# lzhangbj/ASVA

Measured on AMD Instinct MI355X. Metric: UNet denoising steps/sec, 12x256x256 bf16, CFG on, higher is better.
Workload: dtype bf16; 1 GPU; BASELINE configs[1]: AVSync15 shape, 1 clip(s) per GPU per forward, 12x256x256 (latent 12x32x32), SD1.5-shaped AudioUNet3D 1.17B params random-init, CFG batch 2 (audio guidance 4.0), DDIM-50 schedule, step = UNet forward + guidance + scheduler update; clips_per_gpu=1, unet_batch=2, frames=12, launch=hipGraph replay, parallelism=dp1 (independent clips)

## Files before the change

asva_amd/_lib.py:

```python
from __future__ import annotations

import ctypes as C
import os

import torch

from . import precision as P

_HERE = os.path.dirname(os.path.abspath(__file__))
LIB_PATH = os.environ.get("AVSD_LIB_PATH") or os.path.join(_HERE, "libavsd_hip.so")
LIB_PATHS = {"bf16": LIB_PATH, "fp16": os.environ.get("AVSD_LIB_PATH_F16") or os.path.join(_HERE, "libavsd_hip_f16.so")}

c_void_p, c_int, c_float, c_int64 = C.c_void_p, C.c_int, C.c_float, C.c_int64


class GemmDesc(C.Structure):

    _fields_ = [
        ("A", c_void_p), ("A2", c_void_p), ("W", c_void_p), ("out", c_void_p),
        ("bias", c_void_p), ("rowvec", c_void_p), ("res1", c_void_p), ("res2", c_void_p),
        ("M", C.c_int32), ("N", C.c_int32), ("K", C.c_int32),
        ("lda", C.c_int32), ("lda2", C.c_int32), ("k_split", C.c_int32), ("ldw", C.c_int32),
        ("ldc", C.c_int32), ("ldr1", C.c_int32), ("ldr2", C.c_int32),
        ("rows_per_vec", C.c_int32), ("ldv", C.c_int32),
# ... 14 lines not shown


class XAttnDesc(C.Structure):

    _fields_ = [
        ("h", c_void_p), ("ldh", C.c_int32), ("res_f32", C.c_int32),
        ("res", c_void_p), ("ldres", C.c_int32),
        ("M", C.c_int32), ("C", C.c_int32), ("heads", C.c_int32), ("L", C.c_int32),
        ("ln_stats", c_void_p), ("ln_eps", C.c_float), ("scale", C.c_float),
        ("wq", c_void_p), ("ldwq", C.c_int32), ("lk", C.c_int32),
        ("q_colsum", c_void_p), ("q_bias", c_void_p),
        ("k", c_void_p), ("vt", c_void_p),
        ("lk_pad", C.c_int32), ("q_per_kv", C.c_int32),
        ("wo", c_void_p), ("ldwo", C.c_int32), ("ldo", C.c_int32),
        ("o_bias", c_void_p), ("out", c_void_p),
        ("out_master", c_void_p), ("ldm", C.c_int32), ("reserved0", C.c_int32),
        ("rowstats", c_void_p),
        ("stats_pos", c_void_p), ("pos_hw", C.c_int32), ("pos_frames", C.c_int32),
    ]


SIGNATURES = {
    "avsd_abi_version": (c_int, []),
    "avsd_precision": (C.c_char_p, []),
    "avsd_last_error": (C.c_char_p, []),
    "avsd_device_info": (c_int, [C.c_char_p, c_int, C.POINTER(c_int)]),
    "avsd_gemm_bf16": (c_int, [C.POINTER(GemmDesc), c_void_p]),
    "avsd_sizeof_gemm_desc": (c_int, []),
    "avsd_cross_attention_block": (c_int, [C.POINTER(XAttnDesc), c_void_p]),
    "avsd_gemm_conv3r_supported": (c_int, [c_int, c_int, c_int, c_int]),
    "avsd_gemm_conv3r2d_supported": (c_int, [c_int, c_int, c_int, c_int]),
    "avsd_cross_attention_block_supported": (c_int, [c_int, c_int, c_int]),
    "avsd_sizeof_xattn_desc": (c_int, []),
    "avsd_linear_small_m": (c_int, [c_void_p, c_void_p, c_void_p, c_void_p, c_int, c_int, c_int, c_int, c_int, c_int, c_void_p]),
    "avsd_groupnorm_stats": (c_int, [c_void_p, c_int, c_int, c_void_p, c_int, c_int, c_int, c_int, c_int, c_void_p, c_int, c_void_p]),
    "avsd_groupnorm_apply": (c_int, [c_void_p, c_int, c_int, c_void_p, c_int, c_int, c_int, c_int, c_int, c_void_p, c_void_p, c_float,
                                     c_void_p, c_int, c_int, c_void_p, c_int, c_void_p]),
    "avsd_ln_fold": (c_int, [c_void_p, c_int, c_int, c_void_p, c_void_p]),
    "avsd_groupnorm_fused_supported": (c_int, [c_int, c_int, c_int, c_int, c_int, c_int]),
    "avsd_groupnorm_fused": (c_int, [c_void_p, c_int, c_int, c_void_p, c_int, c_int, c_int, c_int, c_int, c_void_p, c_void_p, c_float,
                                     c_int, c_void_p, c_int, c_void_p]),
    "avsd_groupnorm_nchunks": (c_int, [c_int, c_int, c_int]),
    "avsd_groupnorm_scratch_floats": (c_int, [c_int, c_int, c_int, c_int]),
    "avsd_layernorm": (c_int, [c_void_p, c_int, c_void_p, c_int, c_int, c_int, c_void_p, c_void_p, c_float, c_void_p, c_int, c_int, c_void_p]),
    "avsd_softmax_rows": (c_int, [c_void_p, c_int, c_void_p, c_int, c_int, c_int, c_void_p]),
    "avsd_attention": (c_int, [c_void_p, c_int, c_void_p, c_int, c_void_p, c_int, c_void_p, c_int, c_int, c_int, c_int, c_int,
                               c_int, c_int, c_int, c_void_p, c_int, c_float, c_void_p]),
    "avsd_attention_fp8": (c_int, [c_void_p, c_int, c_void_p, c_int, c_void_p, c_int, c_void_p, c_int, c_int, c_int, c_int, c_int,
                                   c_int, c_int, c_int, c_void_p, c_int, c_float, c_float, c_float, c_float, c_void_p]),
    "avsd_temporal_attention": (c_int, [c_void_p, c_int, c_void_p, c_int, c_int, c_int, c_int, c_int, c_int, c_float, c_void_p]),
    "avsd_ncfhw_to_rows": (c_int, [c_void_p, c_void_p, c_int, c_int, c_int, c_int, c_int, c_int, c_float, c_void_p]),
    "avsd_rows_to_ncfhw": (c_int, [c_void_p, c_int, c_void_p, c_int, c_int, c_int, c_int, c_void_p]),
    "avsd_timestep_embedding": (c_int, [c_void_p, c_void_p, c_int, c_int, c_void_p]),
    "avsd_guided_step": (c_int, [c_void_p, c_int, c_float, c_float, c_void_p, c_int, c_float, C.POINTER(C.c_int32), C.POINTER(C.c_float),
                                 c_int, c_void_p, c_void_p, c_float, c_float, c_int, c_int, c_int, c_int, c_void_p]),
    "avsd_guided_multistep": (c_int, [c_void_p, c_int, c_float, c_float, c_void_p, c_int, C.POINTER(C.c_int32), C.POINTER(C.c_float),
                                      c_int, c_void_p, c_void_p, c_float, c_float, c_float, c_float, c_int, c_int, c_int, c_int, c_void_p]),
    "avsd_vae_postprocess":(c_int, [c_void_p, c_int, c_void_p, c_int, c_int, c_void_p]),
    "avsd_vae_postprocess_u8": (c_int, [c_void_p, c_int, c_void_p, c_int, c_int, c_void_p]),
    "avsd_kaldi_fbank": (c_int, [c_void_p, c_int, c_int, C.c_int64, c_void_p, c_void_p, c_int, c_int, c_int, c_int, c_float, c_int,
                                 c_void_p, c_int, c_float, c_float, c_void_p]),
    "avsd_resample_sinc_f32": (c_int, [c_void_p, c_int, c_int, c_int64, c_void_p, c_int, c_int, c_int, c_void_p, c_int, c_int64, c_void_p]),
    "avsd_patchify": (c_int, [c_void_p, c_void_p, c_int, c_int, c_int, c_int, c_int, c_int, c_int, c_void_p]),
    "avsd_vit_tokens": (c_int, [c_void_p, c_void_p, c_void_p, c_void_p, c_int, c_int, c_int, c_int, c_void_p]),
    "avsd_copy": (c_int, [c_void_p, c_void_p, c_int64, c_int, c_void_p]),
    "avsd_xattn_pack_kv": (c_int, [c_void_p, c_int, c_int, c_int, c_void_p, c_int, c_int, c_void_p, c_void_p, c_int, c_void_p]),
# ... 99 lines not shown
```

asva_amd/build.py:

```python
from __future__ import annotations

import os
import subprocess
import sys
from concurrent.futures import ThreadPoolExecutor

HERE = os.path.dirname(os.path.abspath(__file__))
CSRC = os.path.join(HERE, "csrc")
OBJ = os.path.join(CSRC, "_obj")
LIB = os.path.join(HERE, "libavsd_hip.so")
VARIANTS = {"bf16": ("", LIB, []), "fp16": ("_f16", os.path.join(HERE, "libavsd_hip_f16.so"), ["-DAVSD_F16=1"])}
SOURCES = ["lib.hip", "attention.hip", "attention_x2.hip", "gemm_f32.hip", "gemm4.hip", "nstream.hip", "conv3r.hip", "norm.hip", "groupnorm_fused.hip", "elementwise.hip", "audio.hip", "xattn.hip", "attention_fp8.hip", "avsync.hip", "clip_text.hip", "imagebind_eval.hip", "plan.hip"]
GEMM_UNITS = 7
HEADERS = [os.path.join(CSRC, "avsd_common.h"), os.path.join(CSRC, "gemm_common.h"), os.path.join(CSRC, "gemm4_loops.inc"),
           os.path.join(HERE, "..", "include", "avsd.h")]
FLAGS = ["--offload-arch=gfx950", "-O3", "-std=c++17", "-fPIC", "-Wall", "-Wno-unused-function"]


PLAN_HOST = os.path.join(HERE, "plan_host")


def _hipcc() -> str:
    for cand in (os.environ.get("HIPCC"), "/opt/rocm/bin/hipcc", "hipcc"):
        if cand and (os.path.isabs(cand) and os.path.exists(cand) or not os.path.isabs(cand)):
            return cand
    raise RuntimeError("hipcc not found")


def _stale(target: str, deps: list[str]) -> bool:
    if not os.path.exists(target):
        return True
    t = os.path.getmtime(target)
    return any(os.path.getmtime(d) > t for d in deps)


def build(verbose: bool = False, force: bool = False, variants=("bf16", "fp16")) -> str:
    hipcc = _hipcc()
    jobs = []
    links = []
    for var in variants:
        suffix, lib, defs = VARIANTS[var]
        objdir = OBJ + suffix
        os.makedirs(objdir, exist_ok=True)
        objs = []
        stale = False
# ... 39 lines not shown
```

asva_amd/csrc/plan.hip:

```cpp
#include "avsd_common.h"

#include <stdio.h>
#include <string.h>

#include <string>
#include <type_traits>
#include <utility>
#include <vector>

namespace {

struct RArg {
  int64_t i = 0;
  double f = 0.0;
  void* p = nullptr;
};

template <class T>
T conv(const RArg& a) {
  if constexpr (std::is_pointer_v<T>) return reinterpret_cast<T>(a.p);
  else if constexpr (std::is_floating_point_v<T>) return static_cast<T>(a.f);
  else return static_cast<T>(a.i);
}
template <class... A, size_t... I>
int call_impl(int (*fn)(A...), const RArg* a, std::index_sequence<I...>) {
  return fn(conv<A>(a[I])...);
}
template <class... A>
int call(int (*fn)(A...), const RArg* a, int n, const char* name) {
  if (n != (int)sizeof...(A)) {
    avsd_set_error("plan: %s recorded with %d arguments, this library takes %d", name, n, (int)sizeof...(A));
    return AVSD_EINVAL;
  }
  return call_impl(fn, a, std::index_sequence_for<A...>{});
}

typedef int (*thunk_t)(const RArg*, int);
struct Entry {
  const char* name;
  thunk_t thunk;
  size_t desc_bytes;
};
#define AVSD_PLAN_ENTRY(fn) {#fn, [](const RArg* a, int n) { return call(&fn, a, n, #fn); }, 0}
#define AVSD_PLAN_ENTRY_DESC(fn, T) {#fn, [](const RArg* a, int n) { return call(&fn, a, n, #fn); }, sizeof(T)}
const Entry kEntries[] = {
    AVSD_PLAN_ENTRY_DESC(avsd_gemm_bf16, avsd_gemm_desc), AVSD_PLAN_ENTRY_DESC(avsd_cross_attention_block, avsd_xattn_desc), AVSD_PLAN_ENTRY(avsd_linear_small_m),
    AVSD_PLAN_ENTRY(avsd_groupnorm_stats),  AVSD_PLAN_ENTRY(avsd_groupnorm_apply),       AVSD_PLAN_ENTRY(avsd_layernorm),
    AVSD_PLAN_ENTRY(avsd_softmax_rows),     AVSD_PLAN_ENTRY(avsd_attention),             AVSD_PLAN_ENTRY(avsd_attention_fp8),
    AVSD_PLAN_ENTRY(avsd_temporal_attention), AVSD_PLAN_ENTRY(avsd_ncfhw_to_rows),       AVSD_PLAN_ENTRY(avsd_rows_to_ncfhw),
    AVSD_PLAN_ENTRY(avsd_timestep_embedding), AVSD_PLAN_ENTRY(avsd_guided_step),         AVSD_PLAN_ENTRY(avsd_vae_postprocess),
    AVSD_PLAN_ENTRY(avsd_vae_postprocess_u8), AVSD_PLAN_ENTRY(avsd_kaldi_fbank),         AVSD_PLAN_ENTRY(avsd_patchify),
    AVSD_PLAN_ENTRY(avsd_vit_tokens),       AVSD_PLAN_ENTRY(avsd_copy),                  AVSD_PLAN_ENTRY(avsd_xattn_pack_kv),
    AVSD_PLAN_ENTRY(avsd_linear_small_m_x2), AVSD_PLAN_ENTRY(avsd_groupnorm_stats_x2),   AVSD_PLAN_ENTRY(avsd_groupnorm_apply_x2),
    AVSD_PLAN_ENTRY(avsd_layernorm_x2),     AVSD_PLAN_ENTRY(avsd_attention_x2),          AVSD_PLAN_ENTRY(avsd_temporal_attention_x2),
    AVSD_PLAN_ENTRY(avsd_ncfhw_to_rows_x2), AVSD_PLAN_ENTRY(avsd_split_f32),             AVSD_PLAN_ENTRY(avsd_vae_postprocess_x2),
    AVSD_PLAN_ENTRY(avsd_vae_postprocess_u8_x2), AVSD_PLAN_ENTRY(avsd_softmax_rows_x2),
    AVSD_PLAN_ENTRY(avsd_groupnorm_fused),  AVSD_PLAN_ENTRY(avsd_groupnorm_fused_x2),
    AVSD_PLAN_ENTRY(avsd_ln_fold),          AVSD_PLAN_ENTRY(avsd_guided_multistep),
    AVSD_PLAN_ENTRY(avsd_convnd_f32),       AVSD_PLAN_ENTRY(avsd_maxpool_hw_f32),        AVSD_PLAN_ENTRY(avsd_mean_rows_f32),
    AVSD_PLAN_ENTRY(avsd_resize_aa_normalize_f32),
    AVSD_PLAN_ENTRY(avsd_convnd_ld_f32),    AVSD_PLAN_ENTRY(avsd_pool3_hw_f32),
    AVSD_PLAN_ENTRY(avsd_conv3d_same_f32),  AVSD_PLAN_ENTRY(avsd_maxpool3d_same_f32),
    AVSD_PLAN_ENTRY(avsd_embed_tokens_f32), AVSD_PLAN_ENTRY(avsd_layernorm_f32),         AVSD_PLAN_ENTRY(avsd_attention_causal_f32),
    AVSD_PLAN_ENTRY(avsd_quick_gelu_f32),
    AVSD_PLAN_ENTRY(avsd_attention_f32),    AVSD_PLAN_ENTRY(avsd_gelu_f32),              AVSD_PLAN_ENTRY(avsd_vit_tokens_f32),
    AVSD_PLAN_ENTRY(avsd_cosine_rows_f32),   AVSD_PLAN_ENTRY(avsd_normalize_rows_f32),
    AVSD_PLAN_ENTRY(avsd_resample_sinc_f32),
};

struct Reloc {
  uint32_t field_off;
  int32_t buf;
  int64_t off;
};
struct Arg {
  uint8_t tag = 0;
  int64_t i = 0;
  double f = 0.0;
  int32_t buf = -1;
  int64_t off = 0;
  std::vector<unsigned char> blob;
  std::vector<Reloc> relocs;
};
struct Call {
  thunk_t thunk = nullptr;
// ... 352 lines not shown
```

asva_amd/ops.py:

```python
from __future__ import annotations

import os
import ctypes as C
from typing import Optional

import torch

from . import _lib
from . import precision as P
from ._lib import GemmDesc, XAttnDesc, check

PLAIN, TMIX, CONV3 = 0, 1, 2
GEGLU, OUT_F32, GELU, XCD_N, ROWSTATS, LNFUSE, RES1_F32, RES2_F32, X2, KROT, W_FRAG, OUT_REST = 1, 2, 4, 8, 16, 32, 64, 128, 256, 512, 1024, 2048
_XCD_MODE = "auto"
F32 = torch.float32


class KernelTimer:

    def __init__(self):
        self.records = []
        self.replays = []

    def start(self):
# ... 954 lines not shown
    d.h, d.ldh = _p(h), _ld(h)
    _req(res, F32 if res.dtype == F32 else P.ACT, "res")
    d.res, d.ldres, d.res_f32 = _p(res), _ld(res), int(res.dtype == F32)
    d.M, d.C, d.heads, d.L = M, Cc, heads, L
    d.ln_stats, d.ln_eps = _p(stats), float(eps)
    d.scale = float(scale) if scale is not None else float(Cc // heads) ** -0.5
    d.wq, d.ldwq, d.q_colsum, d.q_bias = _p(wq), _ld(wq), _p(q_colsum), _p(q_bias)
    d.k, d.vt, d.lk, d.lk_pad, d.q_per_kv = _p(k), _p(vt), lk, lk_pad, q_per_kv
    d.wo, d.ldwo, d.o_bias = _p(wo), _ld(wo), _p(o_bias)
    d.out, d.ldo = _p(out), _ld(out)
    if master is not None:
        _req(master, F32, "master")
        d.out_master, d.ldm = _p(master), _ld(master)
    if rowstats is not None:
        _req(rowstats, F32, "rowstats")
        d.rowstats = _p(rowstats)
    if stats_pos is not None:
        tbl, hw_, fr_ = stats_pos
        _req(tbl, F32, "stats_pos")
        if rowstats is None or not tbl.is_contiguous() or tbl.shape != (fr_, Cc) or hw_ <= 0:
            raise ValueError("cross_attention_block: stats_pos = (f32 [frames, C], hw, frames) goes with rowstats")
        d.stats_pos, d.pos_hw, d.pos_frames = _p(tbl), int(hw_), int(fr_)
    ev = _TIMER.start() if _TIMER is not None else None
    check(_lib.lib().avsd_cross_attention_block(C.byref(d), _stream()), "avsd_cross_attention_block")
    if ev is not None:
        dc = XAttnDesc.from_buffer_copy(d)
        _TIMER.add_replay("cross_attention_block", lambda dc=dc: check(_lib.lib().avsd_cross_attention_block(C.byref(dc), _stream()),
                                                                         "avsd_cross_attention_block"),
                          (h, stats, wq, q_colsum, q_bias, k, vt, wo, o_bias, res, out, master, rowstats, stats_pos))
        _TIMER.stop(ev, "cross_attention_block", 4.0 * M * Cc * Cc + 4.0 * M * lk * Cc, _nbytes(h, out, res, master) + 4.0 * Cc * Cc)
    return out


def temporal_attention(qkv: torch.Tensor, *, b: int, frames: int, hw: int, heads: int,
                       scale: Optional[float] = None, out: Optional[torch.Tensor] = None) -> torch.Tensor:
    _req(qkv, P.ACT, "qkv")
    Cc = qkv.shape[1] // 3
    d = Cc // heads
    if out is None:
        out = alloc16((qkv.shape[0], Cc), qkv.device)
    if scale is None:
        scale = float(d) ** -0.5
    if P.SPLIT:
        a_ = (_p(qkv), _ld(qkv), _lo(qkv), _p(out), _ld(out), _lo(out), b, frames, hw, heads, d, float(scale))
        call = lambda: check(_lib.lib().avsd_temporal_attention_x2(*a_, _stream()), "avsd_temporal_attention_x2")
    else:
        a_ = (_p(qkv), _ld(qkv), _p(out), _ld(out), b, frames, hw, heads, d, float(scale))
        call = lambda: check(_lib.lib().avsd_temporal_attention(*a_, _stream()), "avsd_temporal_attention")
    _timed("temporal_attention", 4.0 * b * hw * heads * frames * frames * d, _nbytes(qkv, out), (qkv, out), call)
    return out


def ncfhw_to_rows(x: torch.Tensor, cpad: int, rep: int = 1, scale: float = 1.0) -> torch.Tensor:
    _req(x, F32, "x")
    if not x.is_contiguous():
        raise ValueError("ncfhw_to_rows: x must be contiguous")
    B, Cc, Fr, H, W = x.shape
    out = alloc16((rep * B * Fr * H * W, cpad), x.device)
    if P.SPLIT:
        check(_lib.lib().avsd_ncfhw_to_rows_x2(_p(x), _p(out), _lo(out), B, Cc, Fr, H * W, cpad, rep, float(scale), _stream()),
              "avsd_ncfhw_to_rows_x2")
        return out
    check(_lib.lib().avsd_ncfhw_to_rows(_p(x), _p(out), B, Cc, Fr, H * W, cpad, rep, float(scale), _stream()),
          "avsd_ncfhw_to_rows")
    return out

# ... 482 lines not shown
```

asva_amd/plan.py:

```python
from __future__ import annotations

import contextlib
import ctypes as C
import os
import struct
from typing import Dict, List, Optional, Tuple

import torch

from . import _lib
from . import precision as P

CONST, INPUT, OUTPUT = 1, 2, 3
MAGIC = b"AVSDPLN1"
_NOT_RECORDED = {"avsd_abi_version", "avsd_precision", "avsd_last_error", "avsd_device_info", "avsd_sizeof_gemm_desc",
                 "avsd_sizeof_xattn_desc", "avsd_cross_attention_block_supported", "avsd_groupnorm_nchunks",
                 "avsd_groupnorm_scratch_floats", "avsd_groupnorm_fused_supported", "avsd_gemm_conv3r_supported", "avsd_gemm_conv3r2d_supported"}


def _ptr_fields(struct_type) -> List[Tuple[str, int]]:
    return [(name, getattr(struct_type, name).offset) for name, tp in struct_type._fields_ if tp is C.c_void_p]


class _Proxy:

    def __init__(self, real, sink):
        self._real, self._sink = real, sink

    def __getattr__(self, name):
        fn = getattr(self._real, name)
        if (name in _NOT_RECORDED or name.startswith("avsd_plan_") or name.startswith("avsd_unet_") or name == "avsd_vae_decode"
                or name not in _lib.SIGNATURES):
            return fn
        argtypes = _lib.SIGNATURES[name][1]

        def call(*args):
            rc = fn(*args)
            if rc == 0:
                self._sink.append((name, self._convert(name, argtypes, args)))
            return rc

        return call

    @staticmethod
    def _convert(name, argtypes, args):
        out = []
        last = len(argtypes) - 1
        for k, (tp, a) in enumerate(zip(argtypes, args)):
            if tp is C.c_void_p:
# ... 207 lines not shown
```

asva_amd/unet.py:

```python
from __future__ import annotations

import inspect
import json
import math
import os
from typing import Any, Dict, Optional, Tuple, Union

import torch
from torch import nn

from . import precision as P

from . import ops
from .conditioning import mask_to_key_index
from .weights import Blob, _Pk, _Ref, from_act, pack_conv1x1, pack_device, pack_frag, pack_geglu, pack_linear, subpixel_ups, to_act, to_planes

CONFIG_NAME = "config.json"
SAFETENSORS_NAME = "diffusion_pytorch_model.safetensors"
BIN_NAME = "diffusion_pytorch_model.bin"

DOWN_TYPES = ("FFSpatioAudioTempCrossAttnDownBlock3D", "FFSpatioTempCrossAttnDownBlock3D", "FFSpatioTempResDownBlock3D")
UP_TYPES = ("FFSpatioAudioTempCrossAttnUpBlock3D", "FFSpatioTempCrossAttnUpBlock3D", "FFSpatioTempResUpBlock3D")
MID_TYPES = ("FFSpatioAudioTempCrossAttnUNetMidBlock3D", "FFSpatioTempCrossAttnUNetMidBlock3D")


_FUSE_LN = True
_FUSE_LN_TEMP = True
_F32_RES = os.environ.get("AVSD_F32_RESIDUAL", "0") != "0"
_ATTN_FP8 = os.environ.get("AVSD_ATTN_FP8", "0") != "0"
_FUSE_XATTN = True
_LN_PREFOLD = True
_SHARE_PREFIX = True
_F32_CONV_Y = True


def _replicate(a: "_Act", r: int) -> "_Act":
    return _Act(ops.copy(a.lo, rep=r), None if a.hi is None else ops.copy(a.hi, rep=r),
                None if a.rest is None else ops.copy(a.rest, rep=r))


def _xa_fill(kv: torch.Tensor, n_kv: int, rows: int, C: int, idx: Optional[torch.Tensor], old=None):
    nb, lk = (n_kv, rows) if idx is None else (n_kv * idx.shape[0], idx.shape[1])
    lkp = (lk + 31) // 32 * 32
    if lkp > 96 or P.SPLIT:
        return None
    if old is None:
        old = _Pk(k=torch.empty((nb, lkp, C), dtype=kv.dtype, device=kv.device),
                  vt=torch.empty((nb, C, lkp), dtype=kv.dtype, device=kv.device), lk=lk)
    ops.xattn_pack_kv(kv, n_kv, rows, C, idx, old.k, old.vt)
    return old


_FRAME_INDEX: dict = {}
_KEY_INDEX: dict = {}


def key_index_for(mask: torch.Tensor, device) -> torch.Tensor:
    key = (tuple(mask.shape), mask.numpy().tobytes(), str(device))
    if key not in _KEY_INDEX:
        if len(_KEY_INDEX) > 64:
            _KEY_INDEX.clear()
        _KEY_INDEX[key] = mask_to_key_index(mask).to(device)
    return _KEY_INDEX[key]
# ... 879 lines not shown
    C = p.dim
    c = st.cond.blocks[st.tr_i]
    st.tr_i += 1
    n = ops.groupnorm(x.lo, None, B * Fr, L, st.groups, p.norm.g, p.norm.b, 1e-6, False)
    fused = C % 32 == 0 and st.fuse_ln
    eps = 1e-5
    M = B * Fr * L
    stats = [torch.empty((M, C // 32, 2), dtype=torch.float32, device=n.device) for _ in range(2)] if fused else None
    si = 0

    def stream(a, w, bias, res, want_stats=True, stats_pos=None, rest=False):
        nonlocal si
        m = _master(st, a, w.shape[0])
        if fused and want_stats:
            si ^= 1
            return _Act(ops.gemm(a, w, bias=bias, res1=None if res is None else res.res, rowstats=stats[si], master=m, stats_pos=stats_pos), m)
        o16 = o16r = None
        if rest and m is not None:
            o16, o16r = ops.alloc_planes((a.shape[0], w.shape[0]), a.device)
        return _Act(ops.gemm(a, w, bias=bias, res1=None if res is None else res.res, master=m, out=o16, out_rest=o16r), m, o16r)

    def cross(h, a, norm, xa, want_stats, unfused, stats_pos=None):
        nonlocal si
        if fused and st.fp8 is None and xa is not None and ops.cross_attention_block_supported(C, heads, xa.k.shape[1], M, L):
            m = _master(st, h.lo, C)
            s_in = stats[si]
            s_out = None
            if want_stats:
                si ^= 1
                s_out = stats[si]
            out = ops.cross_attention_block(h.lo, s_in, a.wq_ln, a.sq_ln, a.bq_ln, xa.k, xa.vt, xa.lk, a.wo, a.bo, res=h.res,
                                            heads=heads, L=L, q_per_kv=xa.q_per_kv, eps=eps, rowstats=s_out, master=m, stats_pos=stats_pos)
            return _Act(out, m)
        return stream(unfused(), a.wo, a.bo, h, want_stats=want_stats, stats_pos=stats_pos)

    def proj(h, norm, wl, bl, sl, w_plain):
        if fused:
            return ops.gemm(h.lo, wl, bias=bl, ln=(stats[si], sl, eps))
        return ops.gemm(ops.layernorm(h.lo, norm.g, norm.b), w_plain)

    h = stream(n, p.proj_in.w, p.proj_in.b, None)
    a1 = p.attn1
    if fused:
        kv = ops.gemm_batched(h.lo.view(B, Fr * L, C)[:, :L], a1.wkv_ln.unsqueeze(0).expand(B, 2 * C, C), bias=a1.bkv_ln,
                              ln=(stats[si], a1.skv_ln, eps)).view(B * L, 2 * C)
        q = ops.gemm(h.lo, a1.wq_ln, bias=a1.bq_ln, ln=(stats[si], a1.sq_ln, eps))
    else:
        n1 = ops.layernorm(h.lo, p.norm1.g, p.norm1.b)
        q = ops.gemm(n1, a1.wq)
        kv = ops.gemm_batched(n1.view(B, Fr * L, C)[:, :L], a1.wkv.unsqueeze(0).expand(B, 2 * C, C)).view(B * L, 2 * C)
    o = ops.attention(q, kv[:, :C], kv[:, C:], bq=B * Fr, lq=L, lk=L, kv_rows=L, heads=heads, q_per_kv=Fr, frames=Fr, fp8=st.fp8)
    h = stream(o, a1.wo, a1.bo, h)
    if split > 1:
        h, x = _replicate(h, split), _replicate(x, split)
        st.B = B = B * split
        M = B * Fr * L
        if fused:
            cur = stats[si]
            stats = [torch.empty((M, C // 32, 2), dtype=torch.float32, device=n.device) for _ in range(2)]
            ops.copy(cur, stats[si], rep=split)
    if p.audio:
        aa = p.attn_audio

        def audio_attention():
            q = proj(h, p.norm_audio, getattr(aa, "wq_ln", None), getattr(aa, "bq_ln", None), getattr(aa, "sq_ln", None), aa.wq)
            idx = st.cond.key_index
# ... 38 lines not shown
```

include/avsd.h:

```cpp
#ifndef AVSD_H
#define AVSD_H

#include <stddef.h>
#include <stdint.h>

#ifdef __cplusplus
extern "C" {
#endif

#define AVSD_OK 0
#define AVSD_EINVAL (-1)
#define AVSD_ELAUNCH (-2)
#define AVSD_ENODEV (-3)

#define AVSD_ABI_VERSION 10

int avsd_abi_version(void);
const char* avsd_precision(void);
const char* avsd_last_error(void);
int avsd_device_info(char* name_host, int len, int* num_cu_host);

enum { AVSD_GEMM_PLAIN = 0, AVSD_GEMM_TMIX = 1, AVSD_GEMM_CONV3 = 2 };
enum { AVSD_GEMM_GEGLU = 1, AVSD_GEMM_OUT_F32 = 2, AVSD_GEMM_GELU = 4, AVSD_GEMM_XCD_N = 8, AVSD_GEMM_ROWSTATS = 16,
       AVSD_GEMM_LNFUSE = 32, AVSD_GEMM_RES1_F32 = 64, AVSD_GEMM_RES2_F32 = 128, AVSD_GEMM_X2 = 256, AVSD_GEMM_KROT = 512, AVSD_GEMM_W_FRAG = 1024,
// ... 43 lines not shown
  const float* ln_rowvec;
  int32_t pos_hw, pos_frames;
} avsd_gemm_desc;

int avsd_gemm_bf16(const avsd_gemm_desc* desc_host, void* stream);
int avsd_gemm_conv3r_supported(int tile, int hs, int ws, int cin);
int avsd_gemm_conv3r2d_supported(int tile, int hs, int ws, int cin);
int avsd_sizeof_gemm_desc(void);

typedef struct avsd_xattn_desc {
  const void* h;        int32_t ldh;
  int32_t res_f32;
  const void* res;      int32_t ldres;
  int32_t M, C, heads, L;
  const float* ln_stats; float ln_eps;
  float scale;
  const void* wq;       int32_t ldwq;  int32_t lk;
  const float* q_colsum;
  const float* q_bias;
  const void* k;        const void* vt;
  int32_t lk_pad, q_per_kv;
  const void* wo;       int32_t ldwo;  int32_t ldo;
  const float* o_bias;
  void* out;
  float* out_master;    int32_t ldm;   int32_t reserved0;
  float* rowstats;
  const float* stats_pos;
  int32_t pos_hw, pos_frames;
} avsd_xattn_desc;
int avsd_cross_attention_block_supported(int C, int heads, int lk_pad);
int avsd_cross_attention_block(const avsd_xattn_desc* desc_host, void* stream);
int avsd_sizeof_xattn_desc(void);

int avsd_linear_small_m(const float* x, const void* W_bf16, const float* bias, float* out,
                        int M, int N, int K, int ldw, int act_in, int act_out, void* stream);

int avsd_groupnorm_stats(const void* x1, int ld1, int c1, const void* x2, int ld2, int c2,
                         int nb, int rows_per_batch, int groups, float* scratch, int nchunks, void* stream);
int avsd_groupnorm_apply(const void* x1, int ld1, int c1, const void* x2, int ld2, int c2,
                         int nb, int rows_per_batch, int groups, const float* gamma, const float* beta, float eps,
                         const float* scratch, int nchunks, int act, void* y, int ldy, void* stream);
int avsd_groupnorm_fused_supported(int nb, int rows_per_batch, int groups, int c1, int c2, int split);
int avsd_groupnorm_fused(const void* x1, int ld1, int c1, const void* x2, int ld2, int c2, int nb, int rows_per_batch,
                         int groups, const float* gamma, const float* beta, float eps, int act, void* y, int ldy, void* stream);
int avsd_groupnorm_nchunks(int nb, int rows_per_batch, int channels);
int avsd_groupnorm_scratch_floats(int nb, int nchunks, int groups, int channels);

int avsd_ln_fold(const float* stats, int M, int nblk, float* out, void* stream);
int avsd_layernorm(const void* x, int ldx, void* y, int ldy, int M, int C,
                   const float* gamma, const float* beta, float eps,
                   const float* pos, int hw, int frames, void* stream);

int avsd_softmax_rows(const float* S, int lds, void* P, int ldp, int rows, int L, void* stream);

int avsd_attention(const void* Q, int ldq, const void* K, int ldk, const void* V, int ldv,
                   void* O, int ldo, int Bq, int Lq, int Lk, int kv_rows, int heads, int d,
                   int q_per_kv, const int32_t* key_index, int frames, float scale, void* stream);

int avsd_attention_fp8(const void* Q, int ldq, const void* K, int ldk, const void* V, int ldv, void* O, int ldo,
                       int Bq, int Lq, int Lk, int kv_rows, int heads, int d, int q_per_kv,
                       const int32_t* key_index, int frames, float scale, float q_scale, float k_scale,
                       float v_scale, void* stream);

int avsd_temporal_attention(const void* QKV, int ldqkv, void* O, int ldo, int B, int frames,
                            int hw, int heads, int d, float scale, void* stream);

// ... 123 lines not shown
```

Measured before the change: 86.41 steps/s.

## Fuse LayerNorm-folded Q projection with cross-attention into one kernel

Adds a HIP kernel that computes the LayerNorm-folded Q projection GEMM (warp-specialized loader waves with an LDS ring) and then runs cross-attention against preloaded K/V in the same workgroup, writing only the attention output. The unet now uses it for cross-attention blocks that the full cross_attention_block fusion does not cover, with the output projection still a separate stream GEMM. The aim is to avoid writing Q to global memory, reading it back, and paying an extra launch. In exchange each workgroup uses a large LDS footprint and many registers, which may reduce occupancy. The kernel only supports 8 heads, C=640/1280 and lk_pad of 32, 64 or 96.

```diff
diff --git a/asva_amd/_lib.py b/asva_amd/_lib.py
--- a/asva_amd/_lib.py
+++ b/asva_amd/_lib.py
@@ -70,6 +70,8 @@
     "avsd_gemm_conv3r2d_supported": (c_int, [c_int, c_int, c_int, c_int]),
     "avsd_cross_attention_block_supported": (c_int, [c_int, c_int, c_int]),
     "avsd_sizeof_xattn_desc": (c_int, []),
+    "avsd_qproj_attention": (c_int, [C.POINTER(XAttnDesc), c_void_p]),
+    "avsd_qproj_attention_supported": (c_int, [c_int, c_int, c_int, c_int]),
     "avsd_linear_small_m": (c_int, [c_void_p, c_void_p, c_void_p, c_void_p, c_int, c_int, c_int, c_int, c_int, c_int, c_void_p]),
     "avsd_groupnorm_stats": (c_int, [c_void_p, c_int, c_int, c_void_p, c_int, c_int, c_int, c_int, c_int, c_void_p, c_int, c_void_p]),
     "avsd_groupnorm_apply": (c_int, [c_void_p, c_int, c_int, c_void_p, c_int, c_int, c_int, c_int, c_int, c_void_p, c_void_p, c_float,
diff --git a/asva_amd/build.py b/asva_amd/build.py
--- a/asva_amd/build.py
+++ b/asva_amd/build.py
@@ -10,7 +10,7 @@
 OBJ = os.path.join(CSRC, "_obj")
 LIB = os.path.join(HERE, "libavsd_hip.so")
 VARIANTS = {"bf16": ("", LIB, []), "fp16": ("_f16", os.path.join(HERE, "libavsd_hip_f16.so"), ["-DAVSD_F16=1"])}
-SOURCES = ["lib.hip", "attention.hip", "attention_x2.hip", "gemm_f32.hip", "gemm4.hip", "nstream.hip", "conv3r.hip", "norm.hip", "groupnorm_fused.hip", "elementwise.hip", "audio.hip", "xattn.hip", "attention_fp8.hip", "avsync.hip", "clip_text.hip", "imagebind_eval.hip", "plan.hip"]
+SOURCES = ["lib.hip", "attention.hip", "attention_x2.hip", "gemm_f32.hip", "gemm4.hip", "nstream.hip", "conv3r.hip", "norm.hip", "groupnorm_fused.hip", "elementwise.hip", "audio.hip", "xattn.hip", "qattn.hip", "attention_fp8.hip", "avsync.hip", "clip_text.hip", "imagebind_eval.hip", "plan.hip"]
 GEMM_UNITS = 7
 HEADERS = [os.path.join(CSRC, "avsd_common.h"), os.path.join(CSRC, "gemm_common.h"), os.path.join(CSRC, "gemm4_loops.inc"),
            os.path.join(HERE, "..", "include", "avsd.h")]
diff --git a/asva_amd/csrc/plan.hip b/asva_amd/csrc/plan.hip
--- a/asva_amd/csrc/plan.hip
+++ b/asva_amd/csrc/plan.hip
@@ -51,6 +51,7 @@
     AVSD_PLAN_ENTRY(avsd_timestep_embedding), AVSD_PLAN_ENTRY(avsd_guided_step),         AVSD_PLAN_ENTRY(avsd_vae_postprocess),
     AVSD_PLAN_ENTRY(avsd_vae_postprocess_u8), AVSD_PLAN_ENTRY(avsd_kaldi_fbank),         AVSD_PLAN_ENTRY(avsd_patchify),
     AVSD_PLAN_ENTRY(avsd_vit_tokens),       AVSD_PLAN_ENTRY(avsd_copy),                  AVSD_PLAN_ENTRY(avsd_xattn_pack_kv),
+    AVSD_PLAN_ENTRY_DESC(avsd_qproj_attention, avsd_xattn_desc),
     AVSD_PLAN_ENTRY(avsd_linear_small_m_x2), AVSD_PLAN_ENTRY(avsd_groupnorm_stats_x2),   AVSD_PLAN_ENTRY(avsd_groupnorm_apply_x2),
     AVSD_PLAN_ENTRY(avsd_layernorm_x2),     AVSD_PLAN_ENTRY(avsd_attention_x2),          AVSD_PLAN_ENTRY(avsd_temporal_attention_x2),
     AVSD_PLAN_ENTRY(avsd_ncfhw_to_rows_x2), AVSD_PLAN_ENTRY(avsd_split_f32),             AVSD_PLAN_ENTRY(avsd_vae_postprocess_x2),
diff --git a/asva_amd/csrc/qattn.hip b/asva_amd/csrc/qattn.hip
--- /dev/null
+++ b/asva_amd/csrc/qattn.hip
@@ -0,0 +1,389 @@
+#include "avsd_common.h"
+#include "gemm_common.h"
+
+namespace {
+
+struct QAttnArgs {
+  const h16_t* H; int ldh;
+  const h16_t* Wq; int ldwq;
+  const float* q_colsum; const float* q_bias;
+  const float* ln_stats; int ln_nblk; float ln_eps;
+  const h16_t* Kc; const h16_t* Vt;
+  int lk, L, q_per_kv;
+  float sl2;
+  h16_t* O; int ldo;
+  int nwg;
+};
+
+typedef unsigned u32x4 __attribute__((ext_vector_type(4)));
+
+constexpr int QA_NCH = 160;
+
+constexpr int qattn_stages(int BM) { return BM == 64 ? 5 : 4; }
+constexpr int QA_NLW = 4;
+constexpr int QA_CB_BYTES = 2 * QA_NCH * 4;
+constexpr int qattn_threads(int BM) { return (BM / 32 + QA_NLW) * 64; }
+constexpr int qattn_ln_bytes(int BM) { return BM * 8; }
+
+template <int NT>
+constexpr int qattn_lds_bytes(int BM) {
+  const int ring = qattn_stages(BM) * (BM + QA_NCH) * 128;
+  const int kv = NT * 32 * (QA_NCH + 8) * 2 + QA_NCH * (NT * 32 + 4) * 2;
+  return (ring > kv ? ring : kv) + QA_CB_BYTES + qattn_ln_bytes(BM);
+}
+
+template <int C, int D, int BM, int NT>
+__global__ __launch_bounds__(qattn_threads(BM)) void qattn_kernel(const QAttnArgs p) {
+  constexpr int NCW = BM / 32, NLW = QA_NLW, NTHR = (NCW + NLW) * 64;
+  constexpr int NCOL = QA_NCH;
+  constexpr int NG = C / NCOL;
+  constexpr int FN = NCOL / 32;
+  constexpr int HPW = NCOL / D;
+  constexpr int LKP = NT * 32;
+  constexpr int NKT = C / BK;
+  constexpr int A_BYTES = BM * 128, W_BYTES = NCOL * 128, STAGE_BYTES = A_BYTES + W_BYTES;
+  constexpr int PAL = (BM / 8) / NLW, PPL = (STAGE_BYTES / 1024) / NLW;
+  constexpr int NS = qattn_stages(BM);
+  constexpr int RING_BYTES = NS * STAGE_BYTES;
+  constexpr int KS = NCOL + 8;
+  constexpr int VS = LKP + 4;
+  constexpr int SK_BYTES = LKP * KS * 2;
+  static_assert(C % NCOL == 0 && NCOL % D == 0 && D % 16 == 0 && C % BK == 0 && BM % 32 == 0, "shape");
+  static_assert(PAL * NLW * 8 == BM && PPL * NLW * 1024 == STAGE_BYTES && PPL <= 9, "a stage must split evenly into 1-KiB pieces per loader wave");
+  static_assert(SK_BYTES + NCOL * VS * 2 <= RING_BYTES && RING_BYTES + QA_CB_BYTES + qattn_ln_bytes(BM) == qattn_lds_bytes<NT>(BM), "LDS");
+  static_assert(qattn_lds_bytes<NT>(BM) <= 160 * 1024 && NKT >= NS && (NS - 2) * PPL < 64, "ring");
+  extern __shared__ __attribute__((aligned(1024))) unsigned char smq[];
+
+  const int tid = threadIdx.x;
+  const int lane = tid & 63;
+  const int wave = __builtin_amdgcn_readfirstlane(tid >> 6);
+  const bool loader = wave >= NCW;
+  const int lw = wave - NCW;
+  const int half = lane >> 5, l31 = lane & 31, hsel = half * 4;
+  int tm, grp;
+  {
+    const int nwg = p.nwg, bid = blockIdx.x;
+    const int q = nwg >> 3, r = nwg & 7, xcd = bid & 7, idx = bid >> 3;
+    const int w = (xcd < r ? xcd * (q + 1) : r * (q + 1) + (xcd - r) * q) + idx;
+    tm = w / NG;
+    grp = w - tm * NG;
+  }
+  const int row0 = tm * BM;
+  const int ch0 = grp * NCOL;
+  const int kvb = (row0 / p.L) / p.q_per_kv;
+
+  const __amdgpu_buffer_rsrc_t rsH = __builtin_amdgcn_make_buffer_rsrc((void*)p.H, 0, 0x7fffffff, 0x00020000);
+  const __amdgpu_buffer_rsrc_t rsWq = __builtin_amdgcn_make_buffer_rsrc((void*)p.Wq, 0, 0x7fffffff, 0x00020000);
+
+  int poff[9];
+#pragma unroll
+  for (int j = 0; j < PPL; ++j) {
+    int r, kc;
+    if (j < PAL) {
+      piece_row_chunk(lw + j * NLW, lane, r, kc);
+      poff[j] = (row0 + r) * p.ldh + kc;
+    } else {
+      piece_row_chunk(lw + (j - PAL) * NLW, lane, r, kc);
+      poff[j] = (ch0 + r) * p.ldwq + kc;
+    }
+  }
+  const int a_row = (loader ? 0 : wave) * 32 + l31;
+  int w_row[FN];
+#pragma unroll
+  for (int a = 0; a < FN; ++a) w_row[a] = a * 32 + l31;
+
+  f32x16 acc[FN];
+#pragma unroll
+  for (int a = 0; a < FN; ++a)
+#pragma unroll
+    for (int r = 0; r < 16; ++r) acc[a][r] = 0.f;
+
+#define QATTN_ISSUE1(kt_)                                                                                                                  \
+  do {                                                                                                                                    \
+    unsigned char* sb_ = smq + ((kt_) % NS) * STAGE_BYTES + lw * 1024;                                                                    \
+    _Pragma("unroll") for (int j_ = 0; j_ < PPL; ++j_)                                                                                    \
+      __builtin_amdgcn_raw_ptr_buffer_load_lds(j_ < PAL ? rsH : rsWq, (lds_ptr_t)(sb_ + j_ * NLW * 1024), 16, (poff[j_] + (kt_) * BK) * 2, 0, 0, 0); \
+  } while (0)
+  constexpr int KV8 = NCOL / 8, VV8 = LKP / 8;
+  constexpr int NKV = (LKP * KV8 + NTHR - 1) / NTHR, NVV = (NCOL * VV8 + NTHR - 1) / NTHR;
+  u32x4 kreg[NKV], vreg[NVV];
+  {
+    const h16_t* gk = p.Kc + (int64_t)kvb * LKP * C + ch0;
+#pragma unroll
+    for (int u = 0; u < NKV; ++u) {
+      const int v = min(tid + u * NTHR, LKP * KV8 - 1);
+      const int r = v / KV8, c8 = v - r * KV8;
+      kreg[u] = *reinterpret_cast<const u32x4*>(gk + r * C + c8 * 8);
+    }
+    const u32x4* gv = reinterpret_cast<const u32x4*>(p.Vt + ((int64_t)kvb * C + ch0) * LKP);
+#pragma unroll
+    for (int u = 0; u < NVV; ++u) vreg[u] = gv[min(tid + u * NTHR, NCOL * VV8 - 1)];
+  }
+  float* sCB = reinterpret_cast<float*>(smq + RING_BYTES);
+  float2* sLN = reinterpret_cast<float2*>(smq + RING_BYTES + QA_CB_BYTES);
+  if (loader) {
+    const int lt = tid - NCW * 64;
+    constexpr int NB = C / 32, LPR = NLW * 64 / BM, NBL = NB / LPR;
+    static_assert(LPR * BM == NLW * 64 && NBL * LPR == NB && (LPR == 2 || LPR == 4), "statistics split");
+    const float2* st = reinterpret_cast<const float2*>(p.ln_stats) + (int64_t)(row0 + lt / LPR) * p.ln_nblk + (lt % LPR) * NBL;
+    float2 st2[NBL];
+#pragma unroll
+    for (int j = 0; j < NBL; ++j) st2[j] = st[j];
+    const int lc = min(lt, 2 * NCOL / 4 - 1);
+    const float4 cb = *reinterpret_cast<const float4*>((lc < NCOL / 4 ? p.q_colsum : p.q_bias) + ch0 + 4 * (lc % (NCOL / 4)));
+#pragma unroll
+    for (int t = 0; t < NS - 1; ++t) QATTN_ISSUE1(t);
+    *reinterpret_cast<float4*>(sCB + 4 * lc) = cb;
+    float sm = 0.f, sq = 0.f;
+#pragma unroll
+    for (int j = 0; j < NBL; ++j) { sm += st2[j].x; sq += st2[j].y; }
+#pragma unroll
+    for (int o = 1; o < LPR; o *= 2) { sm += __shfl_xor(sm, o, 64); sq += __shfl_xor(sq, o, 64); }
+    const float inv_k = 1.0f / (float)C;
+    const float mean = sm * inv_k;
+    const float rstd = rsqrtf(fmaxf(sq * inv_k - mean * mean, 0.f) + p.ln_eps);
+    if (lt % LPR == 0) sLN[lt / LPR] = make_float2(rstd, mean * rstd);
+  }
+  for (int kt = 0; kt < NKT; ++kt) {
+    if (loader) {
+      wait_tiles_ahead<NS - 2, PPL>(min(NKT - 1, kt + NS - 2) - kt);
+      __builtin_amdgcn_s_waitcnt(0xc07f);
+    }
+    __builtin_amdgcn_s_barrier();
+    if (loader) {
+      if (kt + NS - 1 < NKT) QATTN_ISSUE1(kt + NS - 1);
+    } else {
+      const unsigned char* sA = smq + (kt % NS) * STAGE_BYTES;
+      const unsigned char* sW = sA + A_BYTES;
+#pragma unroll
+      for (int ks = 0; ks < BK / 16; ++ks) {
+        const int c = ks * 2 + half;
+        const h16x8 xf = *reinterpret_cast<const h16x8*>(sA + frag_offset(a_row, c));
+        h16x8 wf[FN];
+#pragma unroll
+        for (int a = 0; a < FN; ++a) wf[a] = *reinterpret_cast<const h16x8*>(sW + frag_offset(w_row[a], c));
+#pragma unroll
+        for (int a = 0; a < FN; ++a) acc[a] = mfma32x32x16(wf[a], xf, acc[a], 0, 0, 0);
+      }
+    }
+  }
+  h16x8 qf[2 * FN];
+  const float2 lnv = sLN[a_row];
+  const float ln_rstd = lnv.x, ln_mr = lnv.y;
+#pragma unroll
+  for (int a = 0; a < (loader ? 0 : FN); ++a) {
+    float v[4][4];
+#pragma unroll
+    for (int q = 0; q < 4; ++q) {
+      const int n = a * 32 + 8 * q + hsel;
+      const float4 cs = *reinterpret_cast<const float4*>(sCB + n);
+      const float4 bb = *reinterpret_cast<const float4*>(sCB + NCOL + n);
+      v[q][0] = fmaf(acc[a][4 * q + 0], ln_rstd, -ln_mr * cs.x) + bb.x;
+      v[q][1] = fmaf(acc[a][4 * q + 1], ln_rstd, -ln_mr * cs.y) + bb.y;
+      v[q][2] = fmaf(acc[a][4 * q + 2], ln_rstd, -ln_mr * cs.z) + bb.z;
+      v[q][3] = fmaf(acc[a][4 * q + 3], ln_rstd, -ln_mr * cs.w) + bb.w;
+    }
+#pragma unroll
+    for (int j = 0; j < 2; ++j) {
+      unsigned e0[2], e1[2];
+#pragma unroll
+      for (int d = 0; d < 2; ++d) {
+        const auto e = __builtin_amdgcn_permlane32_swap(pack2h(v[2 * j][2 * d], v[2 * j][2 * d + 1]),
+                                                        pack2h(v[2 * j + 1][2 * d], v[2 * j + 1][2 * d + 1]), false, false);
+        e0[d] = e[0]; e1[d] = e[1];
+      }
+      qf[2 * a + j] = __builtin_bit_cast(h16x8, make_uint4(e0[0], e0[1], e1[0], e1[1]));
+    }
+  }
+  __syncthreads();
+  unsigned char* sK = smq;
+  unsigned char* sVt = smq + SK_BYTES;
+#pragma unroll
+  for (int u = 0; u < NKV; ++u) {
+    const int v = tid + u * NTHR;
+    if (v < LKP * KV8) {
+      const int r = v / KV8, c8 = v - r * KV8;
+      *reinterpret_cast<u32x4*>(sK + r * (KS * 2) + c8 * 16) = kreg[u];
+    }
+  }
+#pragma unroll
+  for (int u = 0; u < NVV; ++u) {
+    const int v = tid + u * NTHR;
+    if (v < NCOL * VV8) {
+      const int r = v / VV8, k8 = v - r * VV8;
+      uint2* dst = reinterpret_cast<uint2*>(sVt + r * (VS * 2) + k8 * 16);
+      dst[0] = make_uint2(vreg[u].x, vreg[u].y);
+      dst[1] = make_uint2(vreg[u].z, vreg[u].w);
+    }
+  }
+  __syncthreads();
+  if (loader) return;
+
+  f32x16 acc_o[FN];
+#pragma unroll
+  for (int f = 0; f < FN; ++f)
+#pragma unroll
+    for (int r = 0; r < 16; ++r) acc_o[f][r] = 0.f;
+  float inv_l[HPW];
+  const h16x8 zero8 = __builtin_bit_cast(h16x8, make_uint4(0, 0, 0, 0));
+#pragma unroll
+  for (int hh = 0; hh < HPW; ++hh) {
+    constexpr int KBH = D / 16;
+    f32x16 s[NT];
+#pragma unroll
+    for (int t = 0; t < NT; ++t)
+#pragma unroll
+      for (int r = 0; r < 16; ++r) s[t][r] = 0.f;
+#pragma unroll
+    for (int kb = hh * KBH; kb < (hh + 1) * KBH; ++kb) {
+#pragma unroll
+      for (int t = 0; t < NT; ++t) {
+        const h16x8 kf = *reinterpret_cast<const h16x8*>(sK + (32 * t + l31) * (KS * 2) + (16 * kb + 8 * half) * 2);
+        s[t] = mfma32x32x16(kf, qf[kb], s[t], 0, 0, 0);
+      }
+    }
+    float mx = -1e30f;
+#pragma unroll
+    for (int t = 0; t < NT; ++t)
+#pragma unroll
+      for (int r = 0; r < 16; ++r) {
+        const int key = 32 * t + (r & 3) + 8 * (r >> 2) + 4 * half;
+        if (key >= p.lk) s[t][r] = -1e30f;
+        mx = fmaxf(mx, s[t][r]);
+      }
+    mx = fmaxf(mx, __shfl_xor(mx, 32, 64));
+    const float nm = -mx * p.sl2;
+    float psum = 0.f;
+#pragma unroll
+    for (int t = 0; t < NT; ++t)
+#pragma unroll
+      for (int r = 0; r < 16; ++r) {
+        s[t][r] = __builtin_amdgcn_exp2f(fmaf(s[t][r], p.sl2, nm));
+        psum += s[t][r];
+      }
+    psum += __shfl_xor(psum, 32, 64);
+    inv_l[hh] = 1.0f / psum;
+#pragma unroll
+    for (int t = 0; t < NT; ++t)
+#pragma unroll
+      for (int cc = 0; cc < 2; ++cc) {
+        uint4 pv;
+        pv.x = pack2h(s[t][8 * cc + 0], s[t][8 * cc + 1]);
+        pv.y = pack2h(s[t][8 * cc + 2], s[t][8 * cc + 3]);
+        pv.z = pack2h(s[t][8 * cc + 4], s[t][8 * cc + 5]);
+        pv.w = pack2h(s[t][8 * cc + 6], s[t][8 * cc + 7]);
+        const h16x8 pf = __builtin_bit_cast(h16x8, pv);
+#pragma unroll
+        for (int f = 0; f < FN; ++f) {
+          if (32 * f >= D * (hh + 1) || 32 * f + 32 <= D * hh) continue;
+          const int ch = 32 * f + l31;
+          const unsigned char* vr = sVt + ch * (VS * 2) + (32 * t + 16 * cc + 4 * half) * 2;
+          const uint2 lo = *reinterpret_cast<const uint2*>(vr);
+          const uint2 hi = *reinterpret_cast<const uint2*>(vr + 16);
+          h16x8 vv = __builtin_bit_cast(h16x8, make_uint4(lo.x, lo.y, hi.x, hi.y));
+          const bool whole = 32 * f >= D * hh && 32 * f + 32 <= D * (hh + 1);
+          if (!whole && (ch < D * hh || ch >= D * (hh + 1))) vv = zero8;
+          acc_o[f] = mfma32x32x16(vv, pf, acc_o[f], 0, 0, 0);
+        }
+      }
+  }
+
+  h16_t* orow = p.O + (int64_t)(row0 + a_row) * p.ldo + ch0;
+#pragma unroll
+  for (int f = 0; f < FN; ++f) {
+    float v[4][4];
+#pragma unroll
+    for (int q = 0; q < 4; ++q)
+#pragma unroll
+      for (int i = 0; i < 4; ++i) {
+        const int c0 = 32 * f + 8 * q + i;
+        v[q][i] = acc_o[f][4 * q + i] * (half ? inv_l[(c0 + 4) / D] : inv_l[c0 / D]);
+      }
+#pragma unroll
+    for (int j = 0; j < 2; ++j) {
+      unsigned e0[2], e1[2];
+#pragma unroll
+      for (int d = 0; d < 2; ++d) {
+        const auto e = __builtin_amdgcn_permlane32_swap(pack2h(v[2 * j][2 * d], v[2 * j][2 * d + 1]),
+                                                        pack2h(v[2 * j + 1][2 * d], v[2 * j + 1][2 * d + 1]), false, false);
+        e0[d] = e[0]; e1[d] = e[1];
+      }
+      *reinterpret_cast<uint4*>(orow + 32 * f + 16 * j + 8 * half) = make_uint4(e0[0], e0[1], e1[0], e1[1]);
+    }
+  }
+#undef QATTN_ISSUE1
+}
+
+template <int C, int D, int BM, int NT>
+int launch_qattn(QAttnArgs& a, int M, hipStream_t s) {
+  constexpr int lds = qattn_lds_bytes<NT>(BM);
+  static bool attr_set = false;
+  if (!attr_set) {
+    hipError_t e = hipFuncSetAttribute(reinterpret_cast<const void*>(&qattn_kernel<C, D, BM, NT>),
+                                       hipFuncAttributeMaxDynamicSharedMemorySize, lds);
+    if (e != hipSuccess) {
+      avsd_set_error("qproj_attention: hipFuncSetAttribute(%d B LDS): %s", lds, hipGetErrorString(e));
+      return AVSD_ELAUNCH;
+    }
+    attr_set = true;
+  }
+  a.nwg = (M / BM) * (C / QA_NCH);
+  hipLaunchKernelGGL((qattn_kernel<C, D, BM, NT>), dim3((unsigned)a.nwg), dim3(qattn_threads(BM)), (size_t)lds, s, a);
+  AVSD_CHECK_LAUNCH("qproj_attention launch");
+  return AVSD_OK;
+}
+
+template <int C, int D, int BM>
+int launch_qattn_nt(QAttnArgs& a, int M, int lk_pad, hipStream_t s) {
+  switch (lk_pad) {
+    case 32: return launch_qattn<C, D, BM, 1>(a, M, s);
+    case 64: return launch_qattn<C, D, BM, 2>(a, M, s);
+    default: return launch_qattn<C, D, BM, 3>(a, M, s);
+  }
+}
+
+int qattn_bm(int C, int heads, int lk_pad, int rows_per_kv_block) {
+  if (heads != 8 || (lk_pad != 32 && lk_pad != 64 && lk_pad != 96) || rows_per_kv_block <= 0) return 0;
+  if (C == 640) return rows_per_kv_block % 128 == 0 ? 128 : rows_per_kv_block % 64 == 0 ? 64 : 0;
+  if (C == 1280) return rows_per_kv_block % 64 == 0 ? 64 : 0;
+  return 0;
+}
+
+}
+
+extern "C" int avsd_qproj_attention_supported(int C, int heads, int lk_pad, int rows_per_kv_block) {
+  return qattn_bm(C, heads, lk_pad, rows_per_kv_block) ? 1 : 0;
+}
+
+extern "C" int avsd_qproj_attention(const avsd_xattn_desc* dp, void* stream) {
+  AVSD_REQUIRE(dp != nullptr, "qproj_attention: null descriptor");
+  const avsd_xattn_desc& d = *dp;
+  AVSD_REQUIRE(d.h && d.ln_stats && d.wq && d.q_colsum && d.q_bias && d.k && d.vt && d.out, "qproj_attention: null pointer");
+  AVSD_REQUIRE(!d.wo && !d.o_bias && !d.res && !d.rowstats && !d.out_master && !d.stats_pos,
+               "qproj_attention: wo, o_bias, res, rowstats, out_master and stats_pos must be null (the output projection is a launch of its own)");
+  AVSD_REQUIRE(d.L > 0 && d.q_per_kv > 0 && d.M > 0 && d.M % d.L == 0 && (d.M / d.L) % d.q_per_kv == 0,
+               "qproj_attention: M (%d) must be whole K/V blocks of L (%d) x q_per_kv (%d) rows", d.M, d.L, d.q_per_kv);
+  const int64_t rows_per_kv = (int64_t)d.L * d.q_per_kv;
+  const int bm = rows_per_kv <= d.M ? qattn_bm(d.C, d.heads, d.lk_pad, (int)rows_per_kv) : 0;
+  AVSD_REQUIRE(bm != 0,
+               "qproj_attention: unsupported shape C=%d heads=%d lk_pad=%d rows per K/V block=%lld (built: C=640 / 1280, 8 heads, lk_pad 32/64/96, "
+               "K/V blocks of whole 64-row tiles)", d.C, d.heads, d.lk_pad, (long long)rows_per_kv);
+  AVSD_REQUIRE(d.lk > 0 && d.lk <= d.lk_pad, "qproj_attention: bad key count");
+  AVSD_REQUIRE(d.ldh % 8 == 0 && d.ldwq % 8 == 0 && d.ldo % 8 == 0 && d.ldh >= d.C && d.ldwq >= d.C && d.ldo >= d.C,
+               "qproj_attention: row strides must be multiples of 8 and >= C");
+  AVSD_REQUIRE((double)d.M * d.ldh * 2.0 < 2147483648.0 && (double)d.C * d.ldwq * 2.0 < 2147483648.0, "qproj_attention: h and wq must be < 2 GiB");
+  AVSD_REQUIRE(d.scale > 0.f, "qproj_attention: scale must be positive");
+  QAttnArgs a;
+  a.H = (const h16_t*)d.h; a.ldh = d.ldh;
+  a.Wq = (const h16_t*)d.wq; a.ldwq = d.ldwq;
+  a.q_colsum = d.q_colsum; a.q_bias = d.q_bias;
+  a.ln_stats = d.ln_stats; a.ln_nblk = d.C / 32; a.ln_eps = d.ln_eps;
+  a.Kc = (const h16_t*)d.k; a.Vt = (const h16_t*)d.vt;
+  a.lk = d.lk; a.L = d.L; a.q_per_kv = d.q_per_kv;
+  a.sl2 = d.scale * 1.4426950408889634f;
+  a.O = (h16_t*)d.out; a.ldo = d.ldo;
+  a.nwg = 0;
+  hipStream_t s = reinterpret_cast<hipStream_t>(stream);
+  if (d.C == 640) return bm == 128 ? launch_qattn_nt<640, 80, 128>(a, d.M, d.lk_pad, s) : launch_qattn_nt<640, 80, 64>(a, d.M, d.lk_pad, s);
+  return launch_qattn_nt<1280, 160, 64>(a, d.M, d.lk_pad, s);
+}
diff --git a/asva_amd/ops.py b/asva_amd/ops.py
--- a/asva_amd/ops.py
+++ b/asva_amd/ops.py
@@ -1010,6 +1010,56 @@
     return out
 
 
+def qproj_attention_supported(C: int, heads: int, lk_pad: int, M: int, L: int, q_per_kv: int) -> bool:
+    return (not P.SPLIT and L > 0 and q_per_kv > 0 and M % (L * q_per_kv) == 0
+            and bool(_lib.lib().avsd_qproj_attention_supported(C, heads, lk_pad, L * q_per_kv)))
+
+
+def qproj_attention(h: torch.Tensor, stats: torch.Tensor, wq: torch.Tensor, q_colsum: torch.Tensor, q_bias: torch.Tensor,
+                    k: torch.Tensor, vt: torch.Tensor, lk: int, *, heads: int, L: int, q_per_kv: int, eps: float = 1e-5,
+                    scale: Optional[float] = None, out: Optional[torch.Tensor] = None) -> torch.Tensor:
+    if P.SPLIT:
+        raise ValueError("qproj_attention: not built for split precision (use the separate kernels)")
+    _req(h, P.ACT, "h")
+    _req(wq, P.ACT, "wq")
+    _req(k, P.ACT, "k")
+    _req(vt, P.ACT, "vt")
+    _req(stats, F32, "stats")
+    _req(q_colsum, F32, "q_colsum")
+    _req(q_bias, F32, "q_bias")
+    M, Cc = h.shape
+    if k.dim() != 3 or not k.is_contiguous() or not vt.is_contiguous() or vt.shape != (k.shape[0], Cc, k.shape[1]) or k.shape[2] != Cc:
+        raise ValueError("qproj_attention: k must be contiguous [nkv, lk_pad, C] and vt [nkv, C, lk_pad]")
+    lk_pad = k.shape[1]
+    if not stats.is_contiguous() or stats.shape != (M, Cc // 32, 2):
+        raise ValueError("qproj_attention: stats must be contiguous f32 [M, C/32, 2]")
+    if wq.shape != (Cc, Cc) or q_colsum.numel() != Cc or q_bias.numel() != Cc or not q_colsum.is_contiguous() or not q_bias.is_contiguous():
+        raise ValueError("qproj_attention: wq [C, C] with q_colsum [C] and q_bias [C] expected")
+    if L <= 0 or q_per_kv <= 0 or M % L or (M // L) % q_per_kv or (M // L) // q_per_kv > k.shape[0]:
+        raise ValueError("qproj_attention: K/V blocks do not cover the query batches")
+    if out is None:
+        out = torch.empty((M, Cc), dtype=P.ACT, device=h.device)
+    _req(out, P.ACT, "out")
+    if out.shape != (M, Cc):
+        raise ValueError("qproj_attention: out must be [M, C]")
+    d = XAttnDesc()
+    d.h, d.ldh = _p(h), _ld(h)
+    d.M, d.C, d.heads, d.L = M, Cc, heads, L
+    d.ln_stats, d.ln_eps = _p(stats), float(eps)
+    d.scale = float(scale) if scale is not None else float(Cc // heads) ** -0.5
+    d.wq, d.ldwq, d.q_colsum, d.q_bias = _p(wq), _ld(wq), _p(q_colsum), _p(q_bias)
+    d.k, d.vt, d.lk, d.lk_pad, d.q_per_kv = _p(k), _p(vt), lk, lk_pad, q_per_kv
+    d.out, d.ldo = _p(out), _ld(out)
+    ev = _TIMER.start() if _TIMER is not None else None
+    check(_lib.lib().avsd_qproj_attention(C.byref(d), _stream()), "avsd_qproj_attention")
+    if ev is not None:
+        dc = XAttnDesc.from_buffer_copy(d)
+        _TIMER.add_replay("qproj_attention", lambda dc=dc: check(_lib.lib().avsd_qproj_attention(C.byref(dc), _stream()), "avsd_qproj_attention"),
+                          (h, stats, wq, q_colsum, q_bias, k, vt, out))
+        _TIMER.stop(ev, "qproj_attention", 2.0 * M * Cc * Cc + 4.0 * M * lk * Cc, _nbytes(h, out) + 2.0 * Cc * Cc)
+    return out
+
+
 def temporal_attention(qkv: torch.Tensor, *, b: int, frames: int, hw: int, heads: int,
                        scale: Optional[float] = None, out: Optional[torch.Tensor] = None) -> torch.Tensor:
     _req(qkv, P.ACT, "qkv")
diff --git a/asva_amd/plan.py b/asva_amd/plan.py
--- a/asva_amd/plan.py
+++ b/asva_amd/plan.py
@@ -14,7 +14,7 @@
 CONST, INPUT, OUTPUT = 1, 2, 3
 MAGIC = b"AVSDPLN1"
 _NOT_RECORDED = {"avsd_abi_version", "avsd_precision", "avsd_last_error", "avsd_device_info", "avsd_sizeof_gemm_desc",
-                 "avsd_sizeof_xattn_desc", "avsd_cross_attention_block_supported", "avsd_groupnorm_nchunks",
+                 "avsd_sizeof_xattn_desc", "avsd_cross_attention_block_supported", "avsd_qproj_attention_supported", "avsd_groupnorm_nchunks",
                  "avsd_groupnorm_scratch_floats", "avsd_groupnorm_fused_supported", "avsd_gemm_conv3r_supported", "avsd_gemm_conv3r2d_supported"}
 
 
diff --git a/asva_amd/unet.py b/asva_amd/unet.py
--- a/asva_amd/unet.py
+++ b/asva_amd/unet.py
@@ -29,6 +29,7 @@
 _F32_RES = os.environ.get("AVSD_F32_RESIDUAL", "0") != "0"
 _ATTN_FP8 = os.environ.get("AVSD_ATTN_FP8", "0") != "0"
 _FUSE_XATTN = True
+_FUSE_QATTN = os.environ.get("AVSD_FUSE_QATTN", "1") != "0"
 _LN_PREFOLD = True
 _SHARE_PREFIX = True
 _F32_CONV_Y = True
@@ -974,6 +975,12 @@
             out = ops.cross_attention_block(h.lo, s_in, a.wq_ln, a.sq_ln, a.bq_ln, xa.k, xa.vt, xa.lk, a.wo, a.bo, res=h.res,
                                             heads=heads, L=L, q_per_kv=xa.q_per_kv, eps=eps, rowstats=s_out, master=m, stats_pos=stats_pos)
             return _Act(out, m)
+        qa_ok = getattr(ops, "qproj_attention_supported", None)
+        if (_FUSE_QATTN and fused and st.fp8 is None and xa is not None and qa_ok is not None
+                and qa_ok(C, heads, xa.k.shape[1], M, L, xa.q_per_kv)):
+            o = ops.qproj_attention(h.lo, stats[si], a.wq_ln, a.sq_ln, a.bq_ln, xa.k, xa.vt, xa.lk, heads=heads, L=L,
+                                    q_per_kv=xa.q_per_kv, eps=eps)
+            return stream(o, a.wo, a.bo, h, want_stats=want_stats, stats_pos=stats_pos)
         return stream(unfused(), a.wo, a.bo, h, want_stats=want_stats, stats_pos=stats_pos)
 
     def proj(h, norm, wl, bl, sl, w_plain):
diff --git a/include/avsd.h b/include/avsd.h
--- a/include/avsd.h
+++ b/include/avsd.h
@@ -99,6 +99,9 @@
 int avsd_cross_attention_block(const avsd_xattn_desc* desc_host, void* stream);
 int avsd_sizeof_xattn_desc(void);
 
+int avsd_qproj_attention_supported(int C, int heads, int lk_pad, int rows_per_kv_block);
+int avsd_qproj_attention(const avsd_xattn_desc* desc_host, void* stream);
+
 int avsd_linear_small_m(const float* x, const void* W_bf16, const float* bias, float* out,
                         int M, int N, int K, int ldw, int act_in, int act_out, void* stream);
 
```

After: 87.37 steps/s, median of 6. +1.1%, better.
